# GuildOfWeavers/distaff

Measured on AMD Instinct MI355X. Metric: trace_cells_per_sec, higher is better.
Workload: dtype u128 (prime field 2^128-45*2^40+1, 4x u32 limbs)

## Files before the change

distaff_amd/csrc/air_kernel.h:

```cpp
#pragma once
#include "ctx.h"
#include "air_stack_nested.h"

#ifndef AIR_THREADS
#define AIR_THREADS 128
#endif
#ifndef AIR_WAVES_PER_SIMD
#define AIR_WAVES_PER_SIMD 2
#endif

struct AirConsts { fe sponge_mds[16], sponge_inv_mds[16], hasher_mds[36], hasher_inv_mds[36]; };

struct AirArgs {
    const fe* lde;
    fe* out;
    const fe* coef;
    const fe* tc;
    const fe* periodic;
    const AirConsts* consts;
    fe* partial;
    fe* ev[10];
    const fe* tw_lo; const fe* tw_hi; uint32_t lo_bits;
    unsigned long long* bad_step;
    size_t n, col_stride;
    uint32_t log_n, log_N, log_b, W, ctx_depth, loop_depth, stack_depth;
    uint32_t cl, ll, sl;
    uint32_t coset_step;
    uint32_t q0;
    uint32_t num_inputs, num_outputs;
    fe inputs[8], outputs[8], program_hash[2], op_count;
};



__device__ __forceinline__ fe dpow(const AirArgs& a, uint64_t e) {
    uint32_t l = (uint32_t)e & ((1u << a.lo_bits) - 1u), h = (uint32_t)(e >> a.lo_bits);
    fe v = a.tw_lo[l];
    return h ? fe_mul(v, a.tw_hi[h]) : v;
}

template <int Wd>
__device__ __forceinline__ void matmul(fe* s, const fe* m) {
    fe r[Wd];
#pragma unroll
    for (int i = 0; i < Wd; i++) {
        fe_acc A; fe_acc_zero(A);
#pragma unroll
        for (int j = 0; j < Wd; j++) fe_acc_mac(A, m[i * Wd + j], s[j]);
        r[i] = fe_acc_reduce(A);
    }
#pragma unroll
    for (int i = 0; i < Wd; i++) s[i] = r[i];
}

#define AS_BOUNDARY 1
#define AS_OP_BITS 2
#define AS_SPONGE 4
#define AS_STACK_MOVE 8
#define AS_STACK_HIGH 16
#define AS_STACK_ARITH 32
#define AS_STACK_RESCR 64
#define AS_FLOW 128
#define AS_STACK_ANY (AS_STACK_MOVE | AS_STACK_HIGH | AS_STACK_ARITH | AS_STACK_RESCR)
#define AS_STACK_AUX (AS_STACK_MOVE | AS_STACK_ARITH)
#define AF_FIRST 1
#define AF_LAST 2
#define AF_EV_IN 4
#define AF_EV_OUT 8

struct AirStack {
    bool nested, deep;
    int sl;
    int slots;
    int partials;
};
constexpr AirStack air_stack(int sd, int slcap) {
    if (sd == 4) return AirStack{true, false, 8, 4, 6};
    if (sd == 0 && slcap == 8) return AirStack{true, false, 8, 8, 10};
    if (sd == 0 && slcap == 12) return AirStack{true, true, 12, 8, 10};
    return AirStack{false, false, sd ? (sd > 8 ? sd : 8) : slcap, 0, 0};
}

template <uint32_t ACC_MASK>
struct Acc {
    fe_acc res_acc;
    fe_acc adj_acc[6];
    fe res, adj[6];
    bool nonzero;
    const fe* tc; uint32_t nc;
    __device__ __forceinline__ void emit(uint32_t cidx, int slot, const fe& d) {
        nonzero |= !fe_is_zero(d);
        fe_acc_mac(res_acc, d, tc[cidx]);
        if ((ACC_MASK >> slot) & 1u) fe_acc_mac(adj_acc[slot], d, tc[nc + cidx]);
        else adj[slot] = fe_add(adj[slot], fe_mul(d, tc[nc + cidx]));
    }
};
constexpr uint32_t air_acc_mask(const AirStack& st, int sect) { return !st.nested ? 0u : ((sect & AS_OP_BITS) ? 0x01u : 0x3Fu); }

struct AirColumns {
    const fe* cur_p; const fe* nxt_p; size_t cs;
    __device__ __forceinline__ fe cur(size_t c) const { return cur_p[c * cs]; }
    __device__ __forceinline__ fe nxt(size_t c) const { return nxt_p[c * cs]; }
};

template <int CL, int LL>
struct AirRows {
    fe c_opc, n_opc, c_sp[4], n_sp[4], cf[3], n_cf[3], ld[5], hd[2];
    fe c_ctx[CL], n_ctx[CL], c_lp[LL], n_lp[LL];
};

template <int SL, int CL, int LL>
__device__ __forceinline__ void air_load_rows(AirRows<CL, LL>& r, fe* o, fe* nw, const AirArgs& a, const AirColumns p, int sd) {
    r.c_opc = p.cur(0); r.n_opc = p.nxt(0);
#pragma unroll
    for (int i = 0; i < 4; i++) { r.c_sp[i] = p.cur(1 + i); r.n_sp[i] = p.nxt(1 + i); }
#pragma unroll
    for (int i = 0; i < 3; i++) { r.cf[i] = p.cur(5 + i); r.n_cf[i] = p.nxt(5 + i); }
#pragma unroll
    for (int i = 0; i < 5; i++) r.ld[i] = p.cur(8 + i);
#pragma unroll
    for (int i = 0; i < 2; i++) r.hd[i] = p.cur(13 + i);
    uint32_t col = 15;
#pragma unroll
    for (int i = 0; i < CL; i++) { bool on = (uint32_t)i < a.ctx_depth; r.c_ctx[i] = on ? p.cur(col + i) : fe_zero(); r.n_ctx[i] = on ? p.nxt(col + i) : fe_zero(); }
    col += a.ctx_depth;
#pragma unroll
    for (int i = 0; i < LL; i++) { bool on = (uint32_t)i < a.loop_depth; r.c_lp[i] = on ? p.cur(col + i) : fe_zero(); r.n_lp[i] = on ? p.nxt(col + i) : fe_zero(); }
    col += a.loop_depth;
#pragma unroll
    for (int i = 0; i < SL; i++) { bool on = i < sd; o[i] = on ? p.cur(col + i) : fe_zero(); nw[i] = on ? p.nxt(col + i) : fe_zero(); }
}

struct AirFlags {
    fe cff[8], hdf[4], begin_flag, noop_flag, n_void, assert_flag;
    fe lo2[4], mid[4], top[2];
    fe ld_all;
    __device__ __forceinline__ fe ldf(int idx) const { return fe_mul(fe_mul(lo2[idx & 3], mid[(idx >> 2) & 3]), top[idx >> 4]); }
};

__device__ __forceinline__ void air_bit_pairs(fe* t, const fe& a, const fe& na, const fe& nb) {
    t[0] = fe_mul(na, nb); t[1] = fe_sub(nb, t[0]); t[2] = fe_sub(na, t[0]); t[3] = fe_sub(a, t[1]);
}

template <class ROWS>
__device__ __forceinline__ void air_op_flags(AirFlags& f, const ROWS& r) {
    const fe* cf = r.cf; const fe* ld = r.ld; const fe* hd = r.hd;
    {
        fe n0 = bnot(cf[0]), n1 = bnot(cf[1]), n2 = bnot(cf[2]);
        fe t[4];
        air_bit_pairs(t, cf[0], n0, n1);
#pragma unroll
        for (int i = 0; i < 4; i++) { f.cff[i] = fe_mul(t[i], n2); f.cff[4 + i] = fe_sub(t[i], f.cff[i]); }
        f.n_void = fe_mul(fe_mul(r.n_cf[0], r.n_cf[1]), r.n_cf[2]);
        fe l0 = bnot(ld[0]), l1 = bnot(ld[1]), l2 = bnot(ld[2]), l3 = bnot(ld[3]);
        f.lo2[0] = fe_mul(l0, l1); f.lo2[1] = fe_sub(l1, f.lo2[0]);
        f.lo2[2] = fe_mul(l0, cf[1]);
        f.lo2[3] = fe_sub(ld[0], f.lo2[1]);
        air_bit_pairs(f.mid, ld[2], l2, l3);
        f.top[0] = bnot(ld[4]); f.top[1] = ld[4];
        fe h0 = bnot(hd[0]), h1 = bnot(hd[1]);
        air_bit_pairs(f.hdf, hd[0], h0, h1);
    }
    {
        fe ld0 = f.ldf(0);
        f.ld_all = f.ldf(31);
        f.begin_flag = fe_mul(ld0, f.hdf[0]);
        f.noop_flag = fe_mul(f.ld_all, f.hdf[3]);
        f.hdf[0] = fe_mul(f.hdf[0], ld[0]);
        f.assert_flag = fe_mul(ld0, hd[0]);
    }
}

#include "air_stack_perop.h"

template <int CL, int LL, class ROWS>
__device__ __forceinline__ void air_boundary(const AirArgs& a, const ROWS& r, const fe* o, int cl, int ll, uint64_t gi, uint64_t n64, uint64_t nmask, uint32_t ql, size_t k) {
    const fe xp = dpow(a, (gi * (6 * n64 + 2)) & nmask);
    const fe one = fe_one();
#pragma unroll 1
    for (int pass = 0; pass < 2; pass++) {
        const fe* cc = a.coef + pass * 94;
        fe_acc R, A; fe_acc_zero(R); fe_acc_zero(A);
        auto term = [&](const fe& v, uint32_t idx) { fe_acc_mac(R, v, cc[idx]); fe_acc_mac(A, v, cc[idx + 1]); };
        term(pass ? fe_sub(r.c_opc, a.op_count) : r.c_opc, 0);
        if (pass == 0) { for (int i = 0; i < 4; i++) term(r.c_sp[i], 2 + 2 * i); }
        else { for (int i = 0; i < 2; i++) term(fe_sub(r.c_sp[i], a.program_hash[i]), 2 + 2 * i); }
        for (int i = 0; i < 3; i++) term(pass ? fe_sub(r.cf[i], one) : r.cf[i], 10 + 2 * i);
        for (int i = 0; i < 5; i++) term(pass ? fe_sub(r.ld[i], one) : r.ld[i], 16 + 2 * i);
        for (int i = 0; i < 2; i++) term(pass ? fe_sub(r.hd[i], one) : r.hd[i], 26 + 2 * i);
        for (int i = 0; i < CL; i++) if (i < cl) term(r.c_ctx[i], 30 + 2 * i);
        for (int i = 0; i < LL; i++) if (i < ll) term(r.c_lp[i], 62 + 2 * i);
        const uint32_t nio = pass ? a.num_outputs : a.num_inputs;
#pragma unroll
        for (int i = 0; i < 8; i++) if ((uint32_t)i < nio) term(fe_sub(o[i], pass ? a.outputs[i] : a.inputs[i]), 78 + 2 * i);
        const fe adj = fe_acc_reduce(A);
        fe_acc_mac(R, adj, xp);
        a.out[((size_t)pass * gridDim.y + ql) * a.n + k] = fe_acc_reduce(R);
    }
}

template <class ACC, class ROWS>
__device__ __forceinline__ void air_op_bits(ACC& acc, const ROWS& r, const AirFlags& f, const fe* per) {
    const fe* cf = r.cf; const fe* ld = r.ld; const fe* hd = r.hd;
    fe cf_sum = fe_add(fe_add(cf[0], cf[1]), cf[2]);
    const fe ld_prod = f.ld_all, hd_prod = f.hdf[3], all_prod = f.noop_flag;
#pragma unroll
    for (int i = 0; i < 3; i++) acc.emit(i, 0, is_bin(cf[i]));
#pragma unroll
    for (int i = 0; i < 5; i++) acc.emit(3 + i, 0, is_bin(ld[i]));
#pragma unroll
    for (int i = 0; i < 2; i++) acc.emit(8 + i, 0, is_bin(hd[i]));
    const fe is_hacc = f.cff[0];
    acc.emit(10, 1, fe_sub(fe_add(r.c_opc, is_hacc), r.n_opc));
    acc.emit(11, 5, fe_mul(r.c_opc, fe_add(fe_sub(bnot(ld_prod), hd_prod), all_prod)));
    acc.emit(12, 5, fe_mul(cf_sum, bnot(all_prod)));
    acc.emit(13, 3, fe_mul(f.cff[7], bnot(f.n_void)));
    fe prefix = fe_add(fe_add(f.cff[1], f.cff[4]), fe_add(f.cff[5], f.cff[6]));
    fe v = fe_mul(prefix, per[21]);
    v = fe_add(v, fe_mul(fe_add(f.cff[2], f.cff[3]), per[20]));
    v = fe_add(v, fe_mul(f.hdf[0], per[22]));
    acc.emit(14, 2, v);
}

template <bool OWN_CTX, class ACC, class ROWS>
__device__ __forceinline__ void air_sponge(ACC& acc, const AirArgs& a, const AirColumns p, const ROWS& r, const fe* nw, const AirFlags& f, const fe* per) {
    const AirConsts* consts = a.consts;
    fe ctx0;
    if constexpr (OWN_CTX) ctx0 = 0u < a.ctx_depth ? p.cur(15u) : fe_zero();
    else ctx0 = r.c_ctx[0];
    fe sp[4];
    const fe f_begin = f.cff[1], f_tend = f.cff[2], f_fend = f.cff[3], f_loop = f.cff[4], f_wrap = f.cff[5], f_break = f.cff[6], f_void = f.cff[7];
    {
        fe os[4], ns[4];
#pragma unroll
        for (int i = 0; i < 4; i++) os[i] = fe_cube(fe_add(r.c_sp[i], per[i]));
        matmul<4>(os, consts->sponge_mds);
        fe op_code = r.hd[1];
        op_code = fe_add(fe_double(op_code), r.hd[0]);
        op_code = fe_add(fe_double(op_code), r.ld[4]);
        op_code = fe_add(fe_double(op_code), r.ld[3]);
        op_code = fe_add(fe_double(op_code), r.ld[2]);
        op_code = fe_add(fe_double(op_code), r.ld[1]);
        op_code = fe_add(fe_double(op_code), r.ld[0]);
        os[0] = fe_add(os[0], op_code);
        os[1] = fe_add(os[1], fe_mul(nw[0], f.hdf[0]));
#pragma unroll
        for (int i = 0; i < 4; i++) ns[i] = r.n_sp[i];
        matmul<4>(ns, consts->sponge_inv_mds);
#pragma unroll
        for (int i = 0; i < 4; i++) ns[i] = fe_sub(fe_cube(ns[i]), per[4 + i]);
        const fe clr = fe_add(fe_add(f_begin, f_loop), f_wrap);
        const fe cpy = fe_add(f_break, f_void);
        const fe tf = fe_add(f_tend, f_fend);
        const fe xf[4] = {tf, f_tend, f_fend, tf};
        const fe xv[4] = {fe_sub(ctx0, r.n_sp[0]), fe_sub(r.c_sp[0], r.n_sp[1]), fe_sub(r.c_sp[0], r.n_sp[2]), r.n_sp[3]};
#pragma unroll
        for (int i = 0; i < 4; i++) {
            fe_acc A; fe_acc_zero(A);
            fe_acc_mac(A, f.cff[0], fe_sub(os[i], ns[i]));
            fe_acc_mac(A, clr, r.n_sp[i]);
            fe_acc_mac(A, cpy, fe_sub(r.c_sp[i], r.n_sp[i]));
            fe_acc_mac(A, xf[i], xv[i]);
            sp[i] = fe_acc_reduce(A);
        }
    }
    acc.emit(15, 3, sp[0]); acc.emit(16, 4, sp[1]); acc.emit(17, 3, sp[2]); acc.emit(18, 3, sp[3]);
}

template <class CUR>
__device__ __forceinline__ fe air_ctx_constraint(int i, int cl, const fe& push, const fe& pop, const fe& ccpy, const fe& sp0, CUR&& ctx_cur, const fe& ni) {
    fe_acc A; fe_acc_zero(A);
    fe_acc_mac(A, push, fe_sub(i == 0 ? sp0 : ctx_cur(i - 1), ni));
    fe_acc_mac(A, pop, i + 1 < cl ? fe_sub(ctx_cur(i + 1), ni) : ni);
    fe_acc_mac(A, ccpy, fe_sub(ctx_cur(i), ni));
    return fe_acc_reduce(A);
}

template <int CL, int LL, class ACC, class ROWS>
__device__ __forceinline__ void air_flow(ACC& acc, const AirArgs& a, const AirColumns p, const ROWS& r, const AirFlags& f, int cl, int ll) {
    const fe f_begin = f.cff[1], f_tend = f.cff[2], f_fend = f.cff[3], f_loop = f.cff[4], f_wrap = f.cff[5], f_break = f.cff[6], f_void = f.cff[7];
    acc.emit(19, 2, fe_mul(fe_add(f_wrap, f_break), fe_sub(r.c_sp[0], r.c_lp[0])));
    const fe push = fe_add(f_begin, f_loop), pop = fe_add(f_tend, f_fend), ccpy = fe_add(fe_add(f_wrap, f_break), f_void);
    const fe lcpy = fe_add(fe_add(fe_add(f_begin, f_tend), fe_add(f_fend, f_wrap)), f_void);
    if constexpr (CL <= 2 && LL <= 1) {
        auto ctx_cur = [&](int j) { return r.c_ctx[j < 0 ? 0 : (j < CL ? j : 0)]; };
#pragma unroll
        for (int i = 0; i < CL; i++) {
            if (i >= cl) break;
            const fe v = air_ctx_constraint(i, cl, push, pop, ccpy, r.c_sp[0], ctx_cur, r.n_ctx[i]);
            acc.emit(20 + i, 2, v);
        }
#pragma unroll
        for (int i = 0; i < LL; i++) {
            if (i >= ll) break;
            fe v = fe_mul(lcpy, fe_sub(r.c_lp[i], r.n_lp[i]));
            if (i >= 1) v = fe_add(v, fe_mul(f_loop, fe_sub(r.c_lp[i - 1 < 0 ? 0 : i - 1], r.n_lp[i])));
            v = fe_add(v, fe_mul(f_break, i + 1 < ll ? fe_sub(r.c_lp[i + 1 < LL ? i + 1 : 0], r.n_lp[i]) : r.n_lp[i]));
            acc.emit(20 + cl + i, 2, v);
        }
    } else {
        auto ctx_cur = [&](int i) { return (uint32_t)i < a.ctx_depth ? p.cur(15 + i) : fe_zero(); };
        auto ctx_nxt = [&](int i) { return (uint32_t)i < a.ctx_depth ? p.nxt(15 + i) : fe_zero(); };
        const uint32_t lcol = 15 + a.ctx_depth;
        auto lp_cur = [&](int i) { return (uint32_t)i < a.loop_depth ? p.cur(lcol + i) : fe_zero(); };
        auto lp_nxt = [&](int i) { return (uint32_t)i < a.loop_depth ? p.nxt(lcol + i) : fe_zero(); };
#pragma unroll 1
        for (int i = 0; i < cl; i++) {
            const fe ni = ctx_nxt(i);
            acc.emit(20 + i, 2, air_ctx_constraint(i, cl, push, pop, ccpy, r.c_sp[0], ctx_cur, ni));
        }
#pragma unroll 1
        for (int i = 0; i < ll; i++) {
            const fe ni = lp_nxt(i);
            fe_acc A; fe_acc_zero(A);
            fe_acc_mac(A, lcpy, fe_sub(lp_cur(i), ni));
            if (i >= 1) fe_acc_mac(A, f_loop, fe_sub(lp_cur(i - 1), ni));
            fe_acc_mac(A, f_break, i + 1 < ll ? fe_sub(lp_cur(i + 1), ni) : ni);
            acc.emit(20 + cl + i, 2, fe_acc_reduce(A));
        }
    }
}

template <int SD, int NS>
__device__ __forceinline__ void air_rescr_differences(fe* resc, const fe* o, const fe* nw, const fe* per, const AirConsts* consts) {
    constexpr int NZ = (SD != 0 && SD < 6) ? SD : 6;
    fe os[6], ns[6];
#pragma unroll
    for (int i = 0; i < 6; i++) os[i] = i < NZ ? fe_cube(fe_add(o[i], per[8 + i])) : per[23 + i];
    matmul<6>(os, consts->hasher_mds);
    constexpr int NR = NS < 6 ? NS : 6;
#pragma unroll
    for (int i = 0; i < NR; i++) {
        fe_acc A; fe_acc_zero(A);
#pragma unroll
        for (int j = 0; j < NZ; j++) fe_acc_mac(A, consts->hasher_inv_mds[i * 6 + j], nw[j]);
        ns[i] = fe_acc_reduce(A);
    }
#pragma unroll
    for (int i = 0; i < NR; i++) resc[i] = fe_sub(fe_sub(fe_cube(ns[i]), per[14 + i]), os[i]);
}

template <int SD, bool DEEP, int NS, int SL, uint32_t GROUPS, bool EV_IN, bool EV_OUT, class ACC, class ROWS>
__device__ __forceinline__ void air_stack_nested(ACC& acc, const AirArgs& a, const ROWS& r, const fe* o, const fe* nw, const AirFlags& f, const fe* per, int cl, int ll, int sl, int sd, size_t pidx) {
    StackRows rows;
#pragma unroll
    for (int i = 0; i < 8; i++) { rows.o[i] = o[i]; rows.nw[i] = nw[i]; }
#pragma unroll
    for (int i = 8; i < 12; i++) rows.o[i] = DEEP ? o[i < SL ? i : 0] : fe_zero();
    rows.sl = DEEP ? sl : 8;
    const fe lo0h = fe_mul(f.lo2[0], r.hd[0]);
    StackHigh high;
    high.push = f.hdf[0]; high.cmp = f.hdf[1]; high.rescr = f.hdf[2]; high.keep = fe_add(f.begin_flag, f.noop_flag);
    if constexpr ((GROUPS & AG_RESCR) != 0) air_rescr_differences<SD, NS>(high.resc, o, nw, per, a.consts);
    const uint32_t sbase = 20 + cl + ll;
    static_for_air<0, NS + 2>([&](auto k_) {
        constexpr int kk = decltype(k_)::value;
        constexpr int I = kk < NS ? kk : (kk == NS ? ST_AUX0 : ST_AUX1);
        constexpr bool touched = st_touches<I, GROUPS>();
        if constexpr (touched || !EV_OUT) {
            if (I >= 8 || I < sd) {
                fe v = fe_zero();
                if constexpr (touched) v = st_output<I, GROUPS, SD, DEEP>(rows, f.lo2, lo0h, f.mid, f.top, high);
                fe* slot = a.ev[I] + pidx;
                if constexpr (EV_IN) v = touched ? fe_add(v, *slot) : *slot;
                if constexpr (EV_OUT) *slot = v;
                else acc.emit(I >= 8 ? sbase + (I - 8) : sbase + 2 + I, 4, v);
            }
        } else if constexpr (!EV_IN) {
            a.ev[I][pidx] = fe_zero();
        }
    });
}

template <class ACC>
__device__ __forceinline__ void air_stack_deep_slots(ACC& acc, const AirArgs& a, const AirColumns p, const AirFlags& f, int cl, int ll, int sl, int sd) {
    const fe* lo2 = f.lo2; const fe* mid = f.mid; const fe* top = f.top;
    const uint32_t sbase = 20 + cl + ll;
    const fe lo_all = fe_add(fe_add(lo2[0], lo2[1]), fe_add(lo2[2], lo2[3]));
    fe fl1, fl2, fl4, fr1, fr2, fr4, fcp;
    { fe_acc A; fe_acc_zero(A); fe_acc_mac(A, mid[0], lo2[3]); fe_acc_mac(A, mid[2], lo_all); fl1 = fe_add(fe_mul(top[0], fe_acc_reduce(A)), f.assert_flag); }
    { fe_acc A; fe_acc_zero(A); fe_acc_mac(A, mid[0], fe_add(lo2[1], lo2[2])); fe_acc_mac(A, mid[1], fe_add(lo2[1], lo2[3])); fl2 = fe_mul(top[0], fe_acc_reduce(A)); }
    fl4 = fe_mul(top[0], fe_mul(mid[1], fe_add(lo2[0], lo2[2])));
    fr1 = fe_add(fe_mul(top[1], fe_mul(mid[0], fe_add(lo2[0], lo2[2]))), f.hdf[0]);
    { fe_acc A; fe_acc_zero(A); fe_acc_mac(A, mid[0], fe_add(lo2[1], lo2[3])); fe_acc_mac(A, mid[1], lo2[1]); fr2 = fe_mul(top[1], fe_acc_reduce(A)); }
    fr4 = fe_mul(top[1], fe_mul(mid[1], lo2[0]));
    {
        fe_acc A; fe_acc_zero(A); fe_acc_mac(A, mid[2], lo_all); fe_acc_mac(A, mid[3], fe_add(lo2[0], lo2[1]));
        fe_acc B; fe_acc_zero(B); fe_acc_mac(B, top[1], fe_acc_reduce(A)); fe_acc_mac(B, top[0], fe_mul(mid[3], fe_add(fe_add(lo2[0], lo2[1]), lo2[2])));
        fcp = fe_add(fe_add(fe_acc_reduce(B), fe_add(f.hdf[1], f.hdf[2])), fe_add(f.begin_flag, f.noop_flag));
    }
    const uint32_t scol = 15 + a.ctx_depth + a.loop_depth;
#pragma unroll 1
    for (int i = 8; i < sd; i++) {
        const fe ni = p.nxt(scol + i);
        auto item = [&](int j) { return p.cur(scol + j); };
        auto left = [&](int num) { return i + num < sl ? fe_sub(item(i + num), ni) : ni; };
        fe_acc A; fe_acc_zero(A);
        fe_acc_mac(A, fcp, fe_sub(item(i), ni));
        fe_acc_mac(A, fr1, fe_sub(item(i - 1), ni)); fe_acc_mac(A, fr2, fe_sub(item(i - 2), ni)); fe_acc_mac(A, fr4, fe_sub(item(i - 4), ni));
        fe_acc_mac(A, fl1, left(1)); fe_acc_mac(A, fl2, left(2)); fe_acc_mac(A, fl4, left(4));
        acc.emit(sbase + 2 + i, 4, fe_acc_reduce(A));
    }
}

__device__ __forceinline__ void air_combine(const fe& res, const fe* adj, const AirArgs& a, size_t k, uint32_t ql, uint32_t qg, uint64_t gi, uint64_t n64, uint64_t nmask) {
    const bool on_trace = (qg == 0);
    fe t;
    if (on_trace && k + 1 != a.n) {
        t = fe_zero();
    } else {
        const uint32_t degs[6] = {2, 3, 4, 6, 7, 8};
        fe_acc T; fe_acc_zero(T);
        fe_acc_add(T, res);
#pragma unroll
        for (int g = 0; g < 6; g++) {
            uint64_t p = 8 * n64 - 1 - (n64 - 1) * degs[g];
            fe_acc_mac(T, adj[g], dpow(a, (gi * p) & nmask));
        }
        t = fe_acc_reduce(T);
    }
    a.out[((size_t)2 * gridDim.y + ql) * a.n + k] = t;
}

template <int CL, int LL, int SD, int SLCAP, int SECT, uint32_t GROUPS, int FLAGS>
__global__ void __launch_bounds__(AIR_THREADS, AIR_WAVES_PER_SIMD) air_kernel(AirArgs a) {
    constexpr AirStack ST = air_stack(SD, SLCAP);
    constexpr bool FIRST = (FLAGS & AF_FIRST) != 0, LAST = (FLAGS & AF_LAST) != 0, EV_IN = (FLAGS & AF_EV_IN) != 0, EV_OUT = (FLAGS & AF_EV_OUT) != 0;
    static_assert(ST.nested ? (SECT & AS_STACK_ANY) == 0 : (GROUPS == 0 && !EV_IN && !EV_OUT),
                  "nested-sum instances select stack operations with GROUPS, the per-operation instance with SECT");
    const int cl = (int)a.cl, ll = (int)a.ll;
    const int sl = SD ? ST.sl : (int)a.sl;
    const int sd = SD ? SD : (int)a.stack_depth;
    const size_t k = (size_t)blockIdx.x * AIR_THREADS + threadIdx.x;
    if (k >= a.n) return;
    const uint32_t ql = blockIdx.y;
    const uint32_t qg = a.q0 + ql;
    const uint32_t jl = ql * a.coset_step;
    const size_t kn = (k + 1 == a.n) ? 0 : k + 1;
    const AirColumns cols{a.lde + (size_t)jl * a.n + k, a.lde + (size_t)jl * a.n + kn, a.col_stride};
    const uint64_t nmask = ((uint64_t)1 << a.log_N) - 1;
    const uint64_t gi = ((uint64_t)k << a.log_b) + (uint64_t)qg * a.coset_step;
    const uint32_t step = (uint32_t)(((uint64_t)k << 3) + qg);
    const uint64_t n64 = a.n;

    AirRows<CL, LL> rows;
    fe o[ST.sl], nw[ST.sl];
    air_load_rows<ST.sl>(rows, o, nw, a, cols, sd);
    if constexpr ((SECT & AS_BOUNDARY) != 0) air_boundary<CL, LL>(a, rows, o, cl, ll, gi, n64, nmask, ql, k);
    if constexpr (SECT == AS_BOUNDARY) return;
    if (qg == 0 && k + 1 != a.n) {
        if constexpr (LAST) a.out[((size_t)2 * gridDim.y + ql) * a.n + k] = fe_zero();
        return;
    }
    AirFlags flags;
    air_op_flags(flags, rows);
    const fe* per = a.periodic + (size_t)(step & 127u) * AIR_PERIODIC_STRIDE;

    constexpr uint32_t ACC_MASK = air_acc_mask(ST, SECT);
    Acc<ACC_MASK> acc;
#pragma unroll
    for (int i = 0; i < 6; i++) if ((ACC_MASK >> i) & 1u) fe_acc_zero(acc.adj_acc[i]);
    fe_acc_zero(acc.res_acc); acc.res = fe_zero(); acc.nonzero = false; acc.tc = a.tc; acc.nc = 20 + cl + ll + 2 + sd;
#pragma unroll
    for (int i = 0; i < 6; i++) acc.adj[i] = fe_zero();
    const size_t pstride = (size_t)gridDim.y * a.n, pidx = (size_t)ql * a.n + k;

    if constexpr ((SECT & AS_OP_BITS) != 0) air_op_bits(acc, rows, flags, per);
    if constexpr ((SECT & AS_SPONGE) != 0) air_sponge<SD == 0>(acc, a, cols, rows, nw, flags, per);
    if constexpr ((SECT & AS_FLOW) != 0) air_flow<CL, LL>(acc, a, cols, rows, flags, cl, ll);
    if constexpr (ST.nested && (GROUPS & AG_STACK_ALL & ~AG_DEEP) != 0) air_stack_nested<SD, ST.deep, ST.slots, ST.sl, GROUPS, EV_IN, EV_OUT>(acc, a, rows, o, nw, flags, per, cl, ll, sl, sd, pidx);
    if constexpr (!ST.nested && (SECT & AS_STACK_ANY) != 0) air_stack_per_operation<ST.sl, SECT>(acc, o, nw, sl, sd, 20 + cl + ll, flags, per, a.consts);
    if constexpr (ST.deep && (GROUPS & AG_DEEP) != 0) air_stack_deep_slots(acc, a, cols, flags, cl, ll, sl, sd);

    constexpr bool EMITS_STACK = (SECT & AS_STACK_ANY) != 0 || (GROUPS & AG_DEEP) != 0 || ((GROUPS & AG_STACK_ALL) != 0 && !EV_OUT);
    constexpr uint32_t USED = ((SECT & AS_OP_BITS) ? 0x2Fu : 0u) | ((SECT & AS_SPONGE) ? 0x18u : 0u) | ((SECT & AS_FLOW) ? 0x04u : 0u) | (EMITS_STACK ? 0x10u : 0u);
    acc.res = fe_acc_reduce(acc.res_acc);
#pragma unroll
    for (int i = 0; i < 6; i++) if (((ACC_MASK & USED) >> i) & 1u) acc.adj[i] = fe_add(acc.adj[i], fe_acc_reduce(acc.adj_acc[i]));
    if constexpr (!FIRST) {
        acc.res = fe_add(acc.res, a.partial[pidx]);
#pragma unroll
        for (int i = 0; i < 6; i++) if (LAST || ((USED >> i) & 1u)) acc.adj[i] = fe_add(acc.adj[i], a.partial[(size_t)(i + 1) * pstride + pidx]);
    }
    if constexpr (!LAST) {
        a.partial[pidx] = acc.res;
#pragma unroll
        for (int i = 0; i < 6; i++) if (FIRST || ((USED >> i) & 1u)) a.partial[(size_t)(i + 1) * pstride + pidx] = acc.adj[i];
        return;
    }
    air_combine(acc.res, acc.adj, a, k, ql, qg, gi, n64, nmask);
}

struct AirCheckAcc {
    bool nonzero;
    __device__ __forceinline__ void emit(uint32_t, int, const fe& d) { nonzero |= !fe_is_zero(d); }
};

template <int CL, int LL, int SD, int SLCAP, int SECT, uint32_t GROUPS, int FLAGS>
__global__ void __launch_bounds__(AIR_THREADS, AIR_WAVES_PER_SIMD) air_check_kernel(AirArgs a) {
    constexpr AirStack ST = air_stack(SD, SLCAP);
    constexpr bool EV_IN = (FLAGS & AF_EV_IN) != 0, EV_OUT = (FLAGS & AF_EV_OUT) != 0;
    static_assert(ST.nested ? (SECT & AS_STACK_ANY) == 0 : (GROUPS == 0 && !EV_IN && !EV_OUT),
                  "nested-sum instances select stack operations with GROUPS, the per-operation instance with SECT");
    static_assert((SECT & AS_BOUNDARY) == 0, "the boundary combinations are no part of the check");
    const int cl = (int)a.cl, ll = (int)a.ll;
    const int sl = SD ? ST.sl : (int)a.sl;
    const int sd = SD ? SD : (int)a.stack_depth;
    const size_t k = (size_t)blockIdx.x * AIR_THREADS + threadIdx.x;
    if (k + 1 >= a.n) return;
    const AirColumns cols{a.lde + k, a.lde + k + 1, a.col_stride};

    AirRows<CL, LL> rows;
    fe o[ST.sl], nw[ST.sl];
    air_load_rows<ST.sl>(rows, o, nw, a, cols, sd);
    AirFlags flags;
    air_op_flags(flags, rows);
    const fe* per = a.periodic + (size_t)(((uint32_t)k << 3) & 127u) * AIR_PERIODIC_STRIDE;

    AirCheckAcc acc; acc.nonzero = false;
    if constexpr ((SECT & AS_OP_BITS) != 0) air_op_bits(acc, rows, flags, per);
    if constexpr ((SECT & AS_SPONGE) != 0) air_sponge<SD == 0>(acc, a, cols, rows, nw, flags, per);
    if constexpr ((SECT & AS_FLOW) != 0) air_flow<CL, LL>(acc, a, cols, rows, flags, cl, ll);
    if constexpr (ST.nested && (GROUPS & AG_STACK_ALL & ~AG_DEEP) != 0) air_stack_nested<SD, ST.deep, ST.slots, ST.sl, GROUPS, EV_IN, EV_OUT>(acc, a, rows, o, nw, flags, per, cl, ll, sl, sd, k);
    if constexpr (!ST.nested && (SECT & AS_STACK_ANY) != 0) air_stack_per_operation<ST.sl, SECT>(acc, o, nw, sl, sd, 20 + cl + ll, flags, per, a.consts);
    if constexpr (ST.deep && (GROUPS & AG_DEEP) != 0) air_stack_deep_slots(acc, a, cols, flags, cl, ll, sl, sd);
    if (acc.nonzero) atomicMin(a.bad_step, (unsigned long long)k);
}

template <int CL, int LL, int SD, int SLCAP, int SECT, uint32_t GROUPS, int FLAGS>
static void launch_air_check(dst_ctx* c, const AirArgs& a, hipStream_t stream) {
    dim3 g((unsigned)((c->n + AIR_THREADS - 1) / AIR_THREADS), 1);
    static char name[64];
    if (!name[0]) snprintf(name, sizeof(name), "air_check<%d,%d,%d,%d,%d,%u,%d>", CL, LL, SD, SLCAP, SECT, (unsigned)GROUPS, FLAGS);
    constexpr int NS = air_stack(SD, SLCAP).partials;
    const double units = c->W + ((FLAGS & AF_EV_IN) ? NS : 0) + ((FLAGS & AF_EV_OUT) ? NS : 0);
    { KScope ks_(c, name, 16.0 * c->n * units, true, 0.0, stream); hipLaunchKernelGGL((air_check_kernel<CL, LL, SD, SLCAP, SECT, GROUPS, FLAGS>), g, dim3(AIR_THREADS), 0, stream, a); }
}

template <int CL, int LL, int SD, int SLCAP, int SECT, uint32_t GROUPS, int FLAGS>
static void launch_air(dst_ctx* c, const AirArgs& a, uint32_t Q) {
    dim3 g((unsigned)((c->n + AIR_THREADS - 1) / AIR_THREADS), Q);
    static char name[64];
    if (!name[0]) snprintf(name, sizeof(name), "air_kernel<%d,%d,%d,%d,%d,%u,%d>", CL, LL, SD, SLCAP, SECT, (unsigned)GROUPS, FLAGS);
    constexpr int NS = air_stack(SD, SLCAP).partials;
    const double units = c->W + ((FLAGS & AF_FIRST) ? 0 : 7) + ((FLAGS & AF_LAST) ? 1 : 7) + ((SECT & AS_BOUNDARY) ? 2 : 0) + ((FLAGS & AF_EV_IN) ? NS : 0) + ((FLAGS & AF_EV_OUT) ? NS : 0);
    { KScope ks_(c, name, 16.0 * c->n * Q * units, true); hipLaunchKernelGGL((air_kernel<CL, LL, SD, SLCAP, SECT, GROUPS, FLAGS>), g, dim3(AIR_THREADS), 0, c->stream, a); }
}
template <int CL, int LL, int SD, int SLCAP>
static void launch_air_boundary(dst_ctx* c, const AirArgs& a, uint32_t Q) {
#if DST_TEST_HOOKS
    if (dst_internal_boundary_by_evaluation(c)) launch_air<CL, LL, SD, SLCAP, AS_BOUNDARY, 0, 0>(c, a, Q);
#endif
}
struct AirEvalChain {
    dst_ctx* c; const AirArgs& a; uint32_t Q;
    template <int CL, int LL, int SD, int SLCAP, int SECT, uint32_t GROUPS, int FLAGS> void run() const { launch_air<CL, LL, SD, SLCAP, SECT, GROUPS, FLAGS>(c, a, Q); }
    template <int CL, int LL, int SD, int SLCAP> void boundary() const { launch_air_boundary<CL, LL, SD, SLCAP>(c, a, Q); }
};
struct AirCheckChain {
    dst_ctx* c; const AirArgs& a; hipStream_t stream;
    template <int CL, int LL, int SD, int SLCAP, int SECT, uint32_t GROUPS, int FLAGS> void run() const { launch_air_check<CL, LL, SD, SLCAP, SECT, GROUPS, FLAGS>(c, a, stream); }
    template <int CL, int LL, int SD, int SLCAP> void boundary() const {}
};
void air_launch_sd4(dst_ctx* c, const AirArgs& a, uint32_t Q);
void air_launch_small(dst_ctx* c, const AirArgs& a, uint32_t Q);
void air_launch_deep(dst_ctx* c, const AirArgs& a, uint32_t Q);
void air_launch_generic(dst_ctx* c, const AirArgs& a, uint32_t Q);
void air_check_sd4(dst_ctx* c, const AirArgs& a, hipStream_t stream);
void air_check_small(dst_ctx* c, const AirArgs& a, hipStream_t stream);
void air_check_deep(dst_ctx* c, const AirArgs& a, hipStream_t stream);
```

distaff_amd/csrc/air_stack_nested.h:

```cpp
#pragma once
#include <hip/hip_runtime.h>
#include <stdint.h>
#include <type_traits>
#include "fe.h"

__device__ __forceinline__ fe bnot(const fe& v) { return fe_sub(fe_one(), v); }
__device__ __forceinline__ fe is_bin(const fe& v) { return fe_sub(fe_sqr(v), v); }

template <int I, int N, class F>
__device__ __forceinline__ void static_for_air(F&& f) {
    if constexpr (I < N) { f(std::integral_constant<int, I>{}); static_for_air<I + 1, N>(f); }
}

struct StackRows { fe o[12], nw[8]; int sl; };
#define ST_AUX0 8
#define ST_AUX1 9

template <int OP, int I> constexpr bool st_has() {
    constexpr bool slot = I < 8, aux0 = I == ST_AUX0, aux1 = I == ST_AUX1;
    switch (OP) {
        case 0x00: case 0x01: case 0x05: case 0x06: case 0x07: return slot || aux0;
        case 0x02: case 0x0E: return slot || aux0;
        case 0x03: case 0x04: case 0x08: case 0x09: case 0x0C: case 0x0D: return slot;
        case 0x0A: case 0x0B: return slot || aux0 || aux1;
        case 0x10: return I >= 1 && slot;
        case 0x11: return I >= 2 && slot;
        case 0x12: case 0x13: case 0x14: case 0x15: return slot;
        case 0x18: return slot && I != 1;
        case 0x19: case 0x1A: case 0x1B: case 0x1C: case 0x1D: return slot;
        default: return false;
    }
}

template <int OP, int I>
__device__ __forceinline__ fe st_term(const StackRows& s) {
    const fe* o = s.o; const fe* nw = s.nw;
    constexpr int i = I < 8 ? I : 0;
    auto L = [&](int num) {
        if (i + num < 8) return fe_sub(o[i + num < 8 ? i + num : 0], nw[i]);
        return i + num < s.sl ? fe_sub(o[i + num < 12 ? i + num : 0], nw[i]) : nw[i];
    };
    auto R = [&](int num) { return fe_sub(o[i - num < 0 ? 0 : i - num], nw[i]); };
    auto C = [&]() { return fe_sub(o[i], nw[i]); };
    auto sel = [&](const fe& c, const fe& x, const fe& y) { return fe_add(y, fe_mul(c, fe_sub(x, y))); };
    if constexpr (OP == 0x00) { if constexpr (I == ST_AUX0) return bnot(o[0]); else return L(1); }
    else if constexpr (OP == 0x01) { if constexpr (I == ST_AUX0) return fe_sub(o[0], o[1]); else return L(2); }
    else if constexpr (OP == 0x02) {
        const fe diff = fe_sub(o[1], o[2]);
        if constexpr (I == ST_AUX0) return fe_mul(nw[0], diff);
        else if constexpr (I == 0) return fe_sub(nw[0], bnot(fe_mul(diff, o[0])));
        else return L(2);
    }
    else if constexpr (OP == 0x03) return L(1);
    else if constexpr (OP == 0x04) return L(4);
    else if constexpr (OP == 0x05) {
        if constexpr (I == ST_AUX0) return is_bin(o[2]);
        else if constexpr (I == 0) return fe_sub(nw[0], sel(o[2], o[0], o[1]));
        else return L(2);
    }
    else if constexpr (OP == 0x06) {
        if constexpr (I == ST_AUX0) return is_bin(o[4]);
        else if constexpr (I == 0) return fe_sub(nw[0], sel(o[4], o[0], o[2]));
        else if constexpr (I == 1) return fe_sub(nw[1], sel(o[4], o[1], o[3]));
        else return L(4);
    }
    else if constexpr (OP == 0x07) {
        if constexpr (I == ST_AUX0) return is_bin(o[4]);
        else if constexpr (I == 0) return fe_sub(nw[0], sel(o[4], o[2], o[0]));
        else if constexpr (I == 1) return fe_sub(nw[1], sel(o[4], o[3], o[1]));
        else if constexpr (I == 2) return fe_sub(nw[2], sel(o[4], o[0], o[2]));
        else if constexpr (I == 3) return fe_sub(nw[3], sel(o[4], o[1], o[3]));
        else return L(2);
    }
    else if constexpr (OP == 0x08) { if constexpr (I == 0) return fe_sub(nw[0], fe_add(o[0], o[1])); else return L(1); }
    else if constexpr (OP == 0x09) { if constexpr (I == 0) return fe_sub(nw[0], fe_mul(o[0], o[1])); else return L(1); }
    else if constexpr (OP == 0x0A) {
        if constexpr (I == ST_AUX0) return is_bin(o[0]);
        else if constexpr (I == ST_AUX1) return is_bin(o[1]);
        else if constexpr (I == 0) return fe_sub(nw[0], fe_mul(o[0], o[1]));
        else return L(1);
    }
    else if constexpr (OP == 0x0B) {
        if constexpr (I == ST_AUX0) return is_bin(o[0]);
        else if constexpr (I == ST_AUX1) return is_bin(o[1]);
        else if constexpr (I == 0) return fe_sub(nw[0], fe_sub(fe_add(o[0], o[1]), fe_mul(o[0], o[1])));
        else return L(1);
    }
    else if constexpr (OP == 0x0C) { if constexpr (I == 0) return fe_sub(fe_one(), fe_mul(nw[0], o[0])); else return C(); }
    else if constexpr (OP == 0x0D) { if constexpr (I == 0) return fe_add(nw[0], o[0]); else return C(); }
    else if constexpr (OP == 0x0E) {
        if constexpr (I == ST_AUX0) return is_bin(o[0]);
        else if constexpr (I == 0) return fe_sub(nw[0], bnot(o[0]));
        else return C();
    }
    else if constexpr (OP == 0x10) return R(1);
    else if constexpr (OP == 0x11) return R(2);
    else if constexpr (OP == 0x12) { if constexpr (I == 0) return fe_sub(nw[0], o[0]); else return R(1); }
    else if constexpr (OP == 0x13) { if constexpr (I < 2) return fe_sub(nw[i], o[i]); else return R(2); }
    else if constexpr (OP == 0x14) { if constexpr (I < 4) return fe_sub(nw[i], o[i]); else return R(4); }
    else if constexpr (OP == 0x15) { if constexpr (I < 2) return nw[i]; else return R(2); }
    else if constexpr (OP == 0x18) { if constexpr (I == 0) return fe_add(fe_sub(nw[0], o[1]), fe_sub(nw[1], o[0])); else return C(); }
    else if constexpr (OP == 0x19) { if constexpr (I < 4) return fe_sub(nw[i], o[i ^ 2]); else return C(); }
    else if constexpr (OP == 0x1A) return fe_sub(nw[i], o[i ^ 4]);
    else if constexpr (OP == 0x1B) { if constexpr (I < 4) return fe_sub(nw[i], o[(i + 3) & 3]); else return C(); }
    else if constexpr (OP == 0x1C) return fe_sub(nw[i], o[(i + 7) & 7]);
    else if constexpr (OP == 0x1D) {
        if constexpr (I == 0) return is_bin(nw[0]);
        else if constexpr (I == 1) return nw[1];
        else if constexpr (I == 2) return fe_sub(nw[2], fe_double(o[2]));
        else if constexpr (I == 3) return fe_sub(nw[3], fe_add(o[3], fe_mul(nw[0], o[2])));
        else return C();
    }
    else return fe_zero();
}

#define AG_LOW(c, b) (1u << ((c) * 4 + (b)))
#define AG_LOW0 0x00Fu
#define AG_LOW1 0x0F0u
#define AG_PUSH 0x100u
#define AG_CMP 0x200u
#define AG_RESCR 0x400u
#define AG_KEEP 0x800u
#define AG_HIGH 0xF00u
#define AG_DEEP 0x1000u
#define AG_STACK_ALL 0x1FFFu

struct StDesc { int kind, j; };
template <int SDK, bool DEEP>
constexpr StDesc st_desc(int op, int I) {
    const bool o4_zero = SDK != 0 && SDK <= 4;
    if (I >= 8) {
        if ((op == 0x0A || op == 0x0B)) return StDesc{5, I == ST_AUX0 ? 100 : 101};
        if ((op == 0x06 || op == 0x07) && o4_zero) return StDesc{0, 0};
        return StDesc{5, -1};
    }
    const int i = I;
    auto diff = [&](int j) { return (SDK != 0 && j >= SDK) ? StDesc{4, 0} : StDesc{1, j}; };
    auto rdiff = [&](int j) { return (SDK != 0 && j >= SDK) ? StDesc{3, 0} : StDesc{2, j}; };
    auto L = [&](int num) { return i + num < 8 ? diff(i + num) : (DEEP ? StDesc{5, -1} : StDesc{3, 0}); };
    auto R = [&](int num) { return diff(i - num < 0 ? 0 : i - num); };
    switch (op) {
        case 0x00: return L(1);
        case 0x01: return L(2);
        case 0x02: return i == 0 ? StDesc{5, -1} : L(2);
        case 0x03: return L(1);
        case 0x04: return L(4);
        case 0x05: return i == 0 ? StDesc{5, -1} : L(2);
        case 0x06: return i < 2 ? (o4_zero ? rdiff(i + 2) : StDesc{5, -1}) : L(4);
        case 0x07: return i < 4 ? (o4_zero ? rdiff(i) : StDesc{5, -1}) : L(2);
        case 0x08: case 0x0B: return i == 0 ? StDesc{5, -1} : L(1);
        case 0x09: case 0x0A: return i == 0 ? StDesc{5, 102} : L(1);
        case 0x0C: case 0x0D: case 0x0E: return i == 0 ? StDesc{5, -1} : diff(i);
        case 0x10: return R(1);
        case 0x11: return R(2);
        case 0x12: return i == 0 ? rdiff(0) : R(1);
        case 0x13: return i < 2 ? rdiff(i) : R(2);
        case 0x14: return i < 4 ? rdiff(i) : R(4);
        case 0x15: return i < 2 ? StDesc{3, 0} : R(2);
        case 0x18: return i == 0 ? StDesc{5, -1} : diff(i);
        case 0x19: return i < 4 ? rdiff(i ^ 2) : diff(i);
        case 0x1A: return rdiff(i ^ 4);
        case 0x1B: return i < 4 ? rdiff((i + 3) & 3) : diff(i);
        case 0x1C: return rdiff((i + 7) & 7);
        case 0x1D: return i == 1 ? StDesc{3, 0} : (i < 4 ? StDesc{5, -1} : diff(i));
        default: return StDesc{0, 0};
    }
}
struct StMerge { int n; int kind[4], j[4], lead[4]; int sgn[4][4]; };
template <int BASE, int I, int SDK, bool DEEP>
constexpr StMerge st_merge() {
    StMerge m{};
    for (int a = 0; a < 4; a++) {
        const StDesc d = st_desc<SDK, DEEP>(BASE + a, I);
        bool has = false;
        switch (a) { case 0: has = st_has<BASE, I>(); break; case 1: has = st_has<BASE + 1, I>(); break; case 2: has = st_has<BASE + 2, I>(); break; default: has = st_has<BASE + 3, I>(); }
        if (!has || d.kind == 0) continue;
        const int cls = d.kind == 5 ? 5 : (d.kind <= 2 ? 1 : 3);
        const int sign = (d.kind == 2 || d.kind == 4) ? -1 : 1;
        int e = -1;
        for (int k = 0; k < m.n; k++) {
            const int kc = m.kind[k] == 5 ? 5 : (m.kind[k] <= 2 ? 1 : 3);
            if (kc != cls) continue;
            if (cls == 3 || (cls == 1 && m.j[k] == d.j) || (cls == 5 && d.j >= 100 && m.j[k] == d.j)) e = k;
        }
        if (e < 0) { e = m.n++; m.kind[e] = d.kind; m.j[e] = d.j; m.lead[e] = a; m.sgn[e][a] = 1; }
        else { const int lead_sign = (m.kind[e] == 2 || m.kind[e] == 4) ? -1 : 1; m.sgn[e][a] = sign * lead_sign; }
    }
    return m;
}

struct StackHigh { fe push, cmp, rescr, keep; fe resc[6]; };

template <int I, uint32_t GROUPS, int SDK>
__device__ __forceinline__ void st_high_degree(fe_acc& outer, const StackRows& s, const StackHigh& h) {
    if constexpr (I < 8) {
        const fe* o = s.o; const fe* nw = s.nw;
        if constexpr (I >= 1 && (GROUPS & AG_PUSH) != 0) fe_acc_mac(outer, h.push, fe_sub(o[I - 1 < 0 ? 0 : I - 1], nw[I]));
        if constexpr ((GROUPS & AG_CMP) != 0) {
            const fe x_bit = nw[1], y_bit = nw[2], not_set = nw[3];
            fe v;
            if constexpr (I == 0) v = is_bin(x_bit);
            else if constexpr (I == 1) v = is_bin(y_bit);
            else if constexpr (I == 2) v = fe_sub(nw[4], fe_add(o[4], fe_mul(SDK ? fe_sub(x_bit, fe_mul(x_bit, y_bit)) : fe_mul(x_bit, bnot(y_bit)), not_set)));
            else if constexpr (I == 3) v = fe_sub(nw[5], fe_add(o[5], fe_mul(SDK ? fe_sub(y_bit, fe_mul(x_bit, y_bit)) : fe_mul(y_bit, bnot(x_bit)), not_set)));
            else if constexpr (I == 4) v = fe_sub(nw[6], fe_add(o[6], fe_mul(y_bit, o[0])));
            else if constexpr (I == 5) v = fe_sub(nw[7], fe_add(o[7], fe_mul(x_bit, o[0])));
            else if constexpr (I == 6) v = fe_sub(not_set, fe_mul(bnot(o[5]), bnot(o[4])));
            else v = fe_sub(fe_double(nw[0]), o[0]);
            fe_acc_mac(outer, h.cmp, v);
        }
        if constexpr ((GROUPS & (AG_RESCR | AG_KEEP)) != 0) {
            const fe keep = fe_sub(o[I < 8 ? I : 0], nw[I < 8 ? I : 0]);
            if constexpr ((GROUPS & AG_RESCR) != 0) { if constexpr (I < 6) fe_acc_mac(outer, h.rescr, h.resc[I < 6 ? I : 0]); else fe_acc_mac(outer, h.rescr, keep); }
            if constexpr ((GROUPS & AG_KEEP) != 0) fe_acc_mac(outer, h.keep, keep);
        }
    }
}

template <int I, uint32_t GROUPS> constexpr bool st_touches() {
    if (I >= 8) return (GROUPS & AG_LOW0) != 0;
    return (GROUPS & (AG_LOW0 | AG_LOW1 | AG_HIGH)) != 0;
}

template <int I, uint32_t GROUPS, int SDK, bool DEEP>
__device__ __forceinline__ fe st_output(const StackRows& s, const fe* lo2, const fe& lo0h, const fe* mid, const fe* top, const StackHigh& h) {
    fe_acc outer; fe_acc_zero(outer);
    static_for_air<0, 2>([&](auto c_) {
        constexpr int c = decltype(c_)::value;
        if constexpr (((GROUPS >> (4 * c)) & 0xFu) != 0) {
            fe_acc middle; fe_acc_zero(middle);
            static_for_air<0, 4>([&](auto b_) {
                constexpr int b = decltype(b_)::value;
                constexpr int base = 4 * b + 16 * c;
                if constexpr ((GROUPS & AG_LOW(c, b)) != 0) {
                    static constexpr StMerge M = st_merge<base, I, SDK, DEEP>();
                    if constexpr (M.n > 0) {
                        fe_acc inner; fe_acc_zero(inner);
                        static_for_air<0, M.n>([&](auto e_) {
                            constexpr int e = decltype(e_)::value;
                            fe cf = (base == 0 && M.lead[e] == 0) ? lo0h : lo2[M.lead[e]];
                            static_for_air<0, 4>([&](auto a_) {
                                constexpr int a = decltype(a_)::value;
                                if constexpr (a != M.lead[e] && M.sgn[e][a] != 0) {
                                    const fe other = (base == 0 && a == 0) ? lo0h : lo2[a];
                                    cf = M.sgn[e][a] > 0 ? fe_add(cf, other) : fe_sub(cf, other);
                                }
                            });
                            constexpr int ii = I < 8 ? I : 0;
                            fe term;
                            if constexpr (M.kind[e] == 1) term = fe_sub(s.o[M.j[e]], s.nw[ii]);
                            else if constexpr (M.kind[e] == 2) term = fe_sub(s.nw[ii], s.o[M.j[e]]);
                            else if constexpr (M.kind[e] == 3) term = s.nw[ii];
                            else if constexpr (M.kind[e] == 4) term = fe_neg(s.nw[ii]);
                            else term = st_term<base + M.lead[e], I>(s);
                            fe_acc_mac(inner, cf, term);
                        });
                        fe_acc_mac(middle, mid[b], fe_acc_reduce(inner));
                    }
                }
            });
            fe_acc_mac(outer, top[c], fe_acc_reduce(middle));
        }
    });
    if constexpr ((GROUPS & AG_HIGH) != 0) st_high_degree<I, GROUPS, SDK>(outer, s, h);
    return fe_acc_reduce(outer);
}
```

Before: 639.4 million.

## Factor stack constraint outputs into shared opcode-class flag sums

Adds compile-time analysis that groups opcodes by identical signed basis-term signatures across stack slots, computes each class's combined flag sum (mid*top times summed low flags) once, and then evaluates selected 'flat' slots as a short dot product of class sums with distinct basis terms. Slots not chosen by the heuristic still use the nested evaluation. The aim is to remove repeated nested multiply-accumulates in the stack AIR evaluation, at the cost of holding class sums live in registers across the output loop, which may raise register pressure.

```diff
diff --git a/distaff_amd/csrc/air_kernel.h b/distaff_amd/csrc/air_kernel.h
--- a/distaff_amd/csrc/air_kernel.h
+++ b/distaff_amd/csrc/air_kernel.h
@@ -321,6 +321,11 @@
     }
 }
 
+template <int SD, bool DEEP, uint32_t GROUPS>
+constexpr uint32_t air_stack_flat() {
+    return st_flat_default<GROUPS, SD, DEEP>();
+}
+
 template <int SD, int NS>
 __device__ __forceinline__ void air_rescr_differences(fe* resc, const fe* o, const fe* nw, const fe* per, const AirConsts* consts) {
     constexpr int NZ = (SD != 0 && SD < 6) ? SD : 6;
@@ -352,15 +357,17 @@
     StackHigh high;
     high.push = f.hdf[0]; high.cmp = f.hdf[1]; high.rescr = f.hdf[2]; high.keep = fe_add(f.begin_flag, f.noop_flag);
     if constexpr ((GROUPS & AG_RESCR) != 0) air_rescr_differences<SD, NS>(high.resc, o, nw, per, a.consts);
+    constexpr uint32_t FLAT = air_stack_flat<SD, DEEP, GROUPS>();
+    StClassSums<st_class_count<GROUPS, SD, DEEP, FLAT>()> classes;
     const uint32_t sbase = 20 + cl + ll;
-    static_for_air<0, NS + 2>([&](auto k_) {
+    auto output = [&](auto k_) {
         constexpr int kk = decltype(k_)::value;
         constexpr int I = kk < NS ? kk : (kk == NS ? ST_AUX0 : ST_AUX1);
         constexpr bool touched = st_touches<I, GROUPS>();
         if constexpr (touched || !EV_OUT) {
             if (I >= 8 || I < sd) {
                 fe v = fe_zero();
-                if constexpr (touched) v = st_output<I, GROUPS, SD, DEEP>(rows, f.lo2, lo0h, f.mid, f.top, high);
+                if constexpr (touched) v = st_output_basis<I, GROUPS, SD, DEEP, FLAT>(rows, classes, f.lo2, lo0h, f.mid, f.top, high);
                 fe* slot = a.ev[I] + pidx;
                 if constexpr (EV_IN) v = touched ? fe_add(v, *slot) : *slot;
                 if constexpr (EV_OUT) *slot = v;
@@ -369,6 +376,15 @@
         } else if constexpr (!EV_IN) {
             a.ev[I][pidx] = fe_zero();
         }
+    };
+    static_for_air<0, NS + 2>([&](auto k_) {
+        constexpr int kk = decltype(k_)::value;
+        if constexpr (((FLAT >> (kk < NS ? kk : (kk == NS ? ST_AUX0 : ST_AUX1))) & 1u) == 0) output(k_);
+    });
+    st_class_sums<GROUPS, SD, DEEP, FLAT>(classes, f.lo2, lo0h, f.mid, f.top);
+    static_for_air<0, NS + 2>([&](auto k_) {
+        constexpr int kk = decltype(k_)::value;
+        if constexpr (((FLAT >> (kk < NS ? kk : (kk == NS ? ST_AUX0 : ST_AUX1))) & 1u) != 0) output(k_);
     });
 }
 
diff --git a/distaff_amd/csrc/air_stack_nested.h b/distaff_amd/csrc/air_stack_nested.h
--- a/distaff_amd/csrc/air_stack_nested.h
+++ b/distaff_amd/csrc/air_stack_nested.h
@@ -2,6 +2,7 @@
 #include <hip/hip_runtime.h>
 #include <stdint.h>
 #include <type_traits>
+#include <utility>
 #include "fe.h"
 
 __device__ __forceinline__ fe bnot(const fe& v) { return fe_sub(fe_one(), v); }
@@ -265,3 +266,171 @@
     if constexpr ((GROUPS & AG_HIGH) != 0) st_high_degree<I, GROUPS, SDK>(outer, s, h);
     return fe_acc_reduce(outer);
 }
+
+#define ST_NB 32
+struct StBasis { int n; int kind[ST_NB], j[ST_NB], lead[ST_NB]; uint32_t pos[ST_NB], neg[ST_NB]; };
+struct StBasisTable {
+    StBasis b[10];
+    int nclass; uint32_t cls[32];
+};
+
+template <int I, int... OP> constexpr uint32_t st_has_mask_of(std::integer_sequence<int, OP...>) { return ((st_has<OP, I>() ? (1u << OP) : 0u) | ...); }
+template <int I> constexpr uint32_t st_has_mask() { return st_has_mask_of<I>(std::make_integer_sequence<int, 32>{}); }
+constexpr uint32_t st_group_ops(uint32_t groups) {
+    uint32_t ops = 0;
+    for (int g = 0; g < 8; g++) if ((groups >> g) & 1u) ops |= 0xFu << (4 * g);
+    return ops;
+}
+
+template <int SDK, bool DEEP>
+constexpr StBasis st_basis(uint32_t ops, int I) {
+    StBasis m{};
+    for (int op = 0; op < 32; op++) {
+        if (!((ops >> op) & 1u)) continue;
+        const StDesc d = st_desc<SDK, DEEP>(op, I);
+        if (d.kind == 0) continue;
+        const int cls = d.kind == 5 ? 5 : (d.kind <= 2 ? 1 : 3);
+        const int sign = (d.kind == 2 || d.kind == 4) ? -1 : 1;
+        int e = -1;
+        for (int k = 0; k < m.n; k++) {
+            const int kc = m.kind[k] == 5 ? 5 : (m.kind[k] <= 2 ? 1 : 3);
+            if (kc != cls) continue;
+            if (cls == 3 || (cls == 1 && m.j[k] == d.j) || (cls == 5 && d.j >= 100 && m.j[k] == d.j)) e = k;
+        }
+        if (e < 0) { e = m.n++; m.kind[e] = d.kind; m.j[e] = d.j; m.lead[e] = op; m.pos[e] = 1u << op; }
+        else {
+            const int lead_sign = (m.kind[e] == 2 || m.kind[e] == 4) ? -1 : 1;
+            if (sign * lead_sign > 0) m.pos[e] |= 1u << op; else m.neg[e] |= 1u << op;
+        }
+    }
+    return m;
+}
+
+template <uint32_t GROUPS, int SDK, bool DEEP, uint32_t FLAT>
+constexpr StBasisTable st_basis_table() {
+    StBasisTable t{};
+    const uint32_t has[10] = {st_has_mask<0>(), st_has_mask<1>(), st_has_mask<2>(), st_has_mask<3>(), st_has_mask<4>(), st_has_mask<5>(), st_has_mask<6>(),
+                              st_has_mask<7>(), st_has_mask<ST_AUX0>(), st_has_mask<ST_AUX1>()};
+    const uint32_t ops = st_group_ops(GROUPS & (AG_LOW0 | AG_LOW1));
+    int sig[32][10] = {};
+    for (int I = 0; I < 10; I++) {
+        if (!((FLAT >> I) & 1u)) continue;
+        t.b[I] = st_basis<SDK, DEEP>(ops & has[I], I);
+        for (int e = 0; e < t.b[I].n; e++)
+            for (int op = 0; op < 32; op++) {
+                if ((t.b[I].pos[e] >> op) & 1u) sig[op][I] = e + 1;
+                if ((t.b[I].neg[e] >> op) & 1u) sig[op][I] = -(e + 1);
+            }
+    }
+    int first[32] = {};
+    for (int op = 0; op < 32; op++) {
+        bool used = false;
+        for (int I = 0; I < 10; I++) used = used || sig[op][I] != 0;
+        if (!used) continue;
+        int k = -1;
+        for (int c = 0; c < t.nclass && k < 0; c++) {
+            bool same = true;
+            for (int I = 0; I < 10; I++) same = same && sig[op][I] == sig[first[c]][I];
+            if (same) k = c;
+        }
+        if (k < 0) { k = t.nclass++; first[k] = op; }
+        t.cls[k] |= 1u << op;
+    }
+    return t;
+}
+template <uint32_t GROUPS, int SDK, bool DEEP, uint32_t FLAT> struct StBasisOf { static constexpr StBasisTable T = st_basis_table<GROUPS, SDK, DEEP, FLAT>(); };
+template <uint32_t GROUPS, int SDK, bool DEEP, uint32_t FLAT> constexpr int st_class_count() { return StBasisOf<GROUPS, SDK, DEEP, FLAT>::T.nclass; }
+
+template <uint32_t GROUPS, int SDK, bool DEEP>
+constexpr uint32_t st_flat_default() {
+    constexpr StBasisTable all = st_basis_table<GROUPS, SDK, DEEP, 0x0FEu>();
+    uint32_t flat = 0;
+    for (int I = 1; I < 8; I++) {
+        int computed = 0, members = 0;
+        for (int e = 0; e < all.b[I].n; e++) {
+            if (all.b[I].kind[e] == 5) computed++;
+            for (int op = 0; op < 32; op++) members += (int)(((all.b[I].pos[e] | all.b[I].neg[e]) >> op) & 1u);
+        }
+        if (all.b[I].n > 0 && computed <= 2 && members > all.b[I].n) flat |= 1u << I;
+    }
+    return flat;
+}
+
+template <int N> struct StClassSums { fe k[N > 0 ? N : 1]; };
+
+template <int BASE, uint32_t OPS>
+__device__ __forceinline__ fe st_lo_sum(const fe* lo2, const fe& lo0h) {
+    fe v = fe_zero(); bool any = false;
+    static_for_air<0, 4>([&](auto a_) {
+        constexpr int a = decltype(a_)::value;
+        if constexpr (((OPS >> a) & 1u) != 0) {
+            const fe x = (BASE == 0 && a == 0) ? lo0h : lo2[a];
+            v = any ? fe_add(v, x) : x; any = true;
+        }
+    });
+    return v;
+}
+template <uint32_t OPS>
+__device__ __forceinline__ fe st_class_sum(const fe* lo2, const fe& lo0h, const fe* mt) {
+    constexpr int ng = ((OPS & 0xFu) != 0) + ((OPS & 0xF0u) != 0) + ((OPS & 0xF00u) != 0) + ((OPS & 0xF000u) != 0) + ((OPS & 0xF0000u) != 0) + ((OPS & 0xF00000u) != 0) +
+                       ((OPS & 0xF000000u) != 0) + ((OPS & 0xF0000000u) != 0);
+    fe_acc sum; fe_acc_zero(sum);
+    fe only = fe_zero();
+    static_for_air<0, 8>([&](auto g_) {
+        constexpr int g = decltype(g_)::value;
+        constexpr uint32_t grp = (OPS >> (4 * g)) & 0xFu;
+        if constexpr (grp != 0) {
+            const fe lo = st_lo_sum<4 * g, grp>(lo2, lo0h);
+            if constexpr (ng == 1) only = fe_mul(mt[g], lo); else fe_acc_mac(sum, mt[g], lo);
+        }
+    });
+    if constexpr (ng == 1) return only; else return fe_acc_reduce(sum);
+}
+template <uint32_t GROUPS, int SDK, bool DEEP, uint32_t FLAT>
+__device__ __forceinline__ void st_class_sums(StClassSums<st_class_count<GROUPS, SDK, DEEP, FLAT>()>& cs, const fe* lo2, const fe& lo0h, const fe* mid, const fe* top) {
+    using B = StBasisOf<GROUPS, SDK, DEEP, FLAT>;
+    fe mt[8];
+    static_for_air<0, 8>([&](auto g_) {
+        constexpr int g = decltype(g_)::value;
+        constexpr bool used = [] { for (int k = 0; k < B::T.nclass; k++) if ((B::T.cls[k] >> (4 * g)) & 0xFu) return true; return false; }();
+        if constexpr (used) mt[g] = fe_mul(mid[g & 3], top[g >> 2]);
+    });
+    static_for_air<0, B::T.nclass>([&](auto k_) {
+        constexpr int k = decltype(k_)::value;
+        cs.k[k] = st_class_sum<B::T.cls[k]>(lo2, lo0h, mt);
+    });
+}
+
+template <int I, uint32_t GROUPS, int SDK, bool DEEP, uint32_t FLAT>
+__device__ __forceinline__ fe st_output_basis(const StackRows& s, const StClassSums<st_class_count<GROUPS, SDK, DEEP, FLAT>()>& cs, const fe* lo2, const fe& lo0h, const fe* mid,
+                                              const fe* top, const StackHigh& h) {
+    if constexpr (((FLAT >> I) & 1u) == 0) return st_output<I, GROUPS, SDK, DEEP>(s, lo2, lo0h, mid, top, h);
+    else {
+        using B = StBasisOf<GROUPS, SDK, DEEP, FLAT>;
+        fe_acc outer; fe_acc_zero(outer);
+        static_for_air<0, B::T.b[I].n>([&](auto e_) {
+            constexpr int e = decltype(e_)::value;
+            constexpr uint32_t pos = B::T.b[I].pos[e], neg = B::T.b[I].neg[e];
+            fe cf = fe_zero(); bool any = false;
+            static_for_air<0, B::T.nclass>([&](auto k_) {
+                constexpr int k = decltype(k_)::value;
+                if constexpr ((B::T.cls[k] & pos) != 0) { cf = any ? fe_add(cf, cs.k[k]) : cs.k[k]; any = true; }
+            });
+            static_for_air<0, B::T.nclass>([&](auto k_) {
+                constexpr int k = decltype(k_)::value;
+                if constexpr ((B::T.cls[k] & neg) != 0) cf = fe_sub(cf, cs.k[k]);
+            });
+            constexpr int ii = I < 8 ? I : 0;
+            constexpr int kind = B::T.b[I].kind[e], j = B::T.b[I].j[e] < 0 ? 0 : (B::T.b[I].j[e] < 12 ? B::T.b[I].j[e] : 0);
+            fe term;
+            if constexpr (kind == 1) term = fe_sub(s.o[j], s.nw[ii]);
+            else if constexpr (kind == 2) term = fe_sub(s.nw[ii], s.o[j]);
+            else if constexpr (kind == 3) term = s.nw[ii];
+            else if constexpr (kind == 4) term = fe_neg(s.nw[ii]);
+            else term = st_term<B::T.b[I].lead[e], I>(s);
+            fe_acc_mac(outer, cf, term);
+        });
+        if constexpr ((GROUPS & AG_HIGH) != 0) st_high_degree<I, GROUPS, SDK>(outer, s, h);
+        return fe_acc_reduce(outer);
+    }
+}
```

New measurement: 646.2 million (median of 6 runs). +1.1%, better.
